# nickmass/mass-raytrace

Hardware: AMD Instinct MI355X
Metric: Msamples/sec (rays traced/sec) at 1920×1080×1024spp; 1/2/4/8-GPU scaling (higher is better)
Workload: dtype f32

## Files before the change

mass-raytrace_amd/csrc/device/layout.h:

```cpp
#pragma once
#include <stdint.h>

#include "nf_bound.h"

namespace mrt {

enum : uint32_t { KIND_BOX = 1, KIND_SPHERE = 2, KIND_TRI = 3, KIND_INST = 4, KIND_MODEL = 5, KIND_VOLUME = 6 };
constexpr uint32_t kBoxFlag = 0x80000000u;
enum : uint32_t { kVolInstance = 1, kVolModel = 2 };
constexpr uint32_t kLdsTag = 0x40000000u;
constexpr uint32_t kIdxMask = 0x3FFFFFFFu;
constexpr uint32_t KIND_END = 0;
enum : uint32_t { TRI_FLAG_ALPHA = 1u, TRI_FLAG_UV = 2u, TRI_FLAG_EVE = 4u };
constexpr uint32_t kTriAlpha = 0x80000000u;
constexpr uint32_t kTriIdMask = 0x0FFFFFFFu;

constexpr uint32_t kNfIdx = 0x0FFFFFFFu;
constexpr uint32_t kNfForceL = 0x10000000u, kNfForceR = 0x20000000u;
constexpr uint32_t kNfPop = 0x0FFFFFFFu;
constexpr int kNfExpMin = -100;
constexpr uint32_t kNfStack = 25u;
constexpr uint32_t kNfWildFew = 16u;
constexpr uint32_t kNoParent = 0xFFFFFFFFu;
constexpr uint32_t kWorldKey = 0x80000000u;
enum : uint32_t { VNF_SPHERE = 0, VNF_TRI = 1, VNF_INST = 2, VNF_MODEL = 3 };

constexpr uint32_t SURF_PROGRAM = 0xFFu;
constexpr uint32_t kSurfStack = 4;
struct GpuSurfOp {
  uint32_t op, tex, arg, pad;
  float color[4];
};
struct GpuSurfRef {
  uint32_t kind, index, len, pad;
  float color[4];
};

struct GpuMaterial {
  uint32_t kind, surf_kind, texture;
  float param;
  float color[4];
  uint32_t left, right;
  uint32_t surf_len;
  uint32_t pad1;
};

constexpr uint32_t kTexBlockW = 8, kTexBlockH = 4;
struct GpuTexture {
  uint32_t width, height, wrap;
  uint32_t offset;
};
MRT_HD uint32_t texel_index(uint32_t tpr, uint32_t x, uint32_t y) {
  return (((y >> 2) * tpr + (x >> 3)) << 5) + ((y & 3u) << 3) + (x & 7u);
}

constexpr uint32_t kTriShadeQuads = 7;

constexpr uint32_t kEveQuads = 5;

struct DevScene {
  const uint32_t* slots;
  uint32_t world_begin, world_end;
  const float* inst_inv;
  const float* inst_fwd;
  const uint32_t* inst_mat;
  const uint32_t* model_mat;
  const float* sph;
  const uint32_t* sph_mat;
  const float* tri_shade;
  const GpuMaterial* materials;
  const GpuTexture* textures;
  const uint32_t* texels;
  uint32_t fast_ok;
  uint32_t n_slots, n_tris, n_sph, n_inst, n_models, n_materials, n_textures, n_texels;
  uint32_t* dbg;
  const float* vol_nid;
  const uint32_t* vol_mat;
  const float* ln_table;
  uint32_t n_vol;
  const GpuSurfOp* surf_ops;
  uint32_t n_surf_ops;
  uint32_t bg_kind;
  float bg_color[4];
  const GpuSurfRef* bg_faces;
  const float* bg_m;
  const uint32_t* slots_tl;
  const uint32_t* tlet;
  uint32_t n_tlet;
  uint32_t tl_world_begin;
  uint32_t nf_ok, nf_world;
  uint32_t nf_wild_root;
  const uint32_t* vnf_leaf;
  uint32_t vnf_base[4];
  uint32_t n_vnf;
  NfBound nfb;
  const float* eve;
  const float* tri_tb;
  uint32_t n_eve;
};

}
```

mass-raytrace_amd/csrc/device/material.h:

```cpp
#pragma once
#include "walk.h"

namespace mrt {

struct Surf {
  V3 point, normal;
  V2 uv;
  bool has_uv, front_face;
  uint32_t material;
};

#if defined(__HIP_DEVICE_COMPILE__)
#define MRT_PIN_LOAD(x) asm volatile("" : "+v"(x))
#else
#define MRT_PIN_LOAD(x) (void)0
#endif

struct EveTex {
  uint32_t normal_occlusion, albedo_roughness, pmdg;
};
MRT_HD const float* eve_record(const DevScene& S, uint32_t rec) {
  return S.eve + (size_t)MRT_IDX(S, rec, S.n_eve, 25) * (kEveQuads * 4);
}
MRT_HD EveTex load_eve_tex(const DevScene& S, uint32_t rec) {
  const float4 q = *reinterpret_cast<const float4*>(eve_record(S, rec));
  return EveTex{f2u(q.x), f2u(q.y), f2u(q.z)};
}
MRT_HD V3 eve_tangent_normal(const DevScene& S, uint32_t rec, V2 uv, LocalCounters& lc) {
  const V4 px = texture_get_f(S, load_eve_tex(S, rec).normal_occlusion, uv, lc);
  const float py = px.y * 2.0f - 1.0f, pw = px.w * 2.0f - 1.0f;
  const float x = (1.0f - py * py) - pw * pw;
  return unit(V3{py, pw, sqrtf(fabsf(x))});
}

template <bool EXT>
MRT_HD Surf resolve_hit(const DevScene& S, V3 o, V3 d, const Hit& h, LocalCounters& lc) {
  Surf s;
  V3 ro = o, rd = d;
  const uint32_t ckind = h.container >> 28, cidx = h.container & 0x0FFFFFFFu;
  V3 f0, f1, f2, f3;
  uint32_t over = MRT_NO_MATERIAL;
  if (ckind == MRT_REF_INSTANCE) {
    V3 c0, c1, c2, c3;
    over = S.inst_mat[MRT_IDX(S, cidx, S.n_inst, 12)];
    load_m12(S.inst_inv + (size_t)MRT_IDX(S, cidx, S.n_inst, 9) * 12, c0, c1, c2, c3);
    ro = xform(c0, c1, c2, c3, o, 1.0f);
    rd = xform(c0, c1, c2, c3, d, 0.0f);
  } else if (ckind == MRT_REF_MODEL) {
    over = S.model_mat[MRT_IDX(S, cidx, S.n_models, 13)];
  }
  const uint32_t pkind = h.prim >> 28, pidx = h.prim & 0x0FFFFFFFu;
  V3 outward;
  s.point = ro + rd * h.t;
  if (pkind == MRT_REF_VOLUME) {
    s.normal = V3{1.0f, 0.0f, 0.0f};
    s.front_face = true;
    s.has_uv = false;
    s.uv = V2{0, 0};
    s.material = S.vol_mat[MRT_IDX(S, pidx, S.n_vol, 16)];
    return s;
  }
  if (pkind == MRT_REF_SPHERE) {
    const uint32_t sp = MRT_IDX(S, pidx, S.n_sph, 10);
    V3 c = ld3(S.sph + (size_t)sp * 4);
    float r = S.sph[(size_t)sp * 4 + 3];
    s.material = S.sph_mat[sp];
    MRT_PIN_LOAD(s.material);
    outward = (s.point - c) / r;
    s.has_uv = false;
    s.uv = V2{0, 0};
  } else {
    TriShade t = load_tri(S, pidx);
    float4 tq{}, bq{};
    if (EXT && S.tri_tb) {
      const float4* tb = reinterpret_cast<const float4*>(S.tri_tb) + (size_t)MRT_IDX(S, pidx, S.n_tris, 3) * 2;
      tq = tb[0], bq = tb[1];
    }
    float a0, a1, a2;
    tri_bary(t, s.point, a0, a1, a2);
    outward = (t.na * a0 + t.nb * a1) + t.nc * a2;
    s.has_uv = (t.flags & TRI_FLAG_UV) != 0;
    s.uv = uv_or_zero(s.has_uv, (t.uva * a0 + t.uvb * a1) + t.uvc * a2);
    s.material = t.material;
    if (EXT && S.tri_tb && s.has_uv && (t.flags & TRI_FLAG_EVE)) {
      const V3 tn = eve_tangent_normal(S, t.eve, s.uv, lc);
      outward = ((V3{tq.x, tq.y, tq.z} * tn.x) + (V3{bq.x, bq.y, bq.z} * tn.y)) + (outward * tn.z);
    }
  }
  s.front_face = dot(rd, outward) < 0.0f;
  s.normal = s.front_face ? outward : -outward;
  if (ckind == MRT_REF_INSTANCE) {
    load_m12(S.inst_fwd + (size_t)MRT_IDX(S, cidx, S.n_inst, 11) * 12, f0, f1, f2, f3);
    s.point = xform(f0, f1, f2, f3, s.point, 1.0f);
    s.normal = unit(xform(f0, f1, f2, f3, s.normal, 0.0f));
  }
  if (over != MRT_NO_MATERIAL) s.material = over;
  return s;
}
MRT_HD Surf resolve_hit(const DevScene& S, V3 o, V3 d, const Hit& h) {
  LocalCounters lc;
  return resolve_hit<false>(S, o, d, h, lc);
}

MRT_DEV V3 random_in_unit_sphere(PathRng& rng) {
  for (;;) {
    float x = rng.f32() * 2.0f - 1.0f;
    float y = rng.f32() * 2.0f - 1.0f;
    float z = rng.f32() * 2.0f - 1.0f;
    V3 v{x, y, z};
    if (length_squared(v) >= 1.0f) continue;
    return v;
  }
}
MRT_DEV V3 random_in_unit_disk(PathRng& rng) {
  for (;;) {
    float x = rng.f32() * 2.0f - 1.0f;
    float y = rng.f32() * 2.0f - 1.0f;
    V3 v{x, y, 0.0f};
    if (length_squared(v) >= 1.0f) continue;
    return v;
  }
}

MRT_DEV float reflectance(float cosine, float ref_idx) {
  float r0 = (1.0f - ref_idx) / (1.0f + ref_idx);
  r0 = r0 * r0;
  float x = 1.0f - cosine;
  return r0 + (1.0f - r0) * (x * ((x * x) * (x * x)));
}

struct DevCamera {
  V3 origin, llc, horizontal, vertical, u, v;
  float lens_radius;
};

MRT_DEV void camera_ray_uv(const DevCamera& cam, float u, float v, PathRng& rng, V3& o, V3& d) {
  V3 blur = random_in_unit_disk(rng) * cam.lens_radius;
  V3 offset = cam.u * blur.x + cam.v * blur.y;
  o = cam.origin + offset;
  d = (((cam.llc + (cam.horizontal * u)) + (cam.vertical * v)) - cam.origin) - offset;
}

MRT_DEV void camera_ray(const DevCamera& cam, uint32_t x, uint32_t y, uint32_t W, uint32_t H, PathRng& rng, V3& o,
                        V3& d) {
  float u = ((float)x + rng.f32()) / (float)(W - 1);
  float v = ((float)y + rng.f32()) / (float)(H - 1);
  camera_ray_uv(cam, u, v, rng, o, d);
}

template <bool EXT>
MRT_DEV V3 background(const DevScene& S, V3 d, LocalCounters& lc) {
  if (S.bg_kind == MRT_BG_SOLID) return V3{S.bg_color[0], S.bg_color[1], S.bg_color[2]};
  if (S.bg_kind == MRT_BG_SKY) {
    V3 ud = unit(d);
    float t = 0.5f * (ud.y + 1.0f);
    return (fill3(1.0f) * (1.0f - t)) + (V3{0.5f, 0.7f, 1.0f} * t);
  }
  V2 uv{0.0f, 0.0f};
  uint32_t face = 0;
  if (!EXT || S.bg_kind == MRT_BG_SKYSPHERE) {
    V3 p = unit(d);
    float theta = acosf(p.y);
    float phi = atan2f(p.z * -1.0f, p.x) + kPi;
    uv = V2{phi / (2.0f * kPi), theta / kPi};
  } else if (EXT) {
    const float* mf = S.bg_m;
    const M4 m{V4{mf[0], mf[1], mf[2], mf[3]}, V4{mf[4], mf[5], mf[6], mf[7]}, V4{mf[8], mf[9], mf[10], mf[11]},
               V4{mf[12], mf[13], mf[14], mf[15]}};
    V3 p = transform(m, d, 0.0f);
    V3 a{fabsf(p.x), fabsf(p.y), fabsf(p.z)};
    float max_axis = 0.0f, u = 0.0f, v = 0.0f;
    if (a.x >= a.y && a.x >= a.z) {
      if (p.x > 0.0f) face = 0, u = p.z * -1.0f, v = p.y;
      else face = 1, u = p.z, v = p.y;
      max_axis = a.x;
    } else if (a.y >= a.x && a.y >= a.z) {
      if (p.y > 0.0f) face = 3, u = p.x, v = p.z * -1.0f;
      else face = 2, u = p.x, v = p.z;
      max_axis = a.y;
    } else if (a.z >= a.x && a.z >= a.y) {
      if (p.z > 0.0f) face = 4, u = p.x, v = p.y;
      else face = 5, u = p.x * -1.0f, v = p.y;
      max_axis = a.z;
    }
    uv = V2{0.5f * (u / max_axis + 1.0f), 0.5f * (v / max_axis + 1.0f)};
  }
  const GpuSurfRef f = S.bg_faces[face];
  V4 px = surface_ref_get_f<EXT>(S, f.kind, f.index, f.len, f.color, uv, lc);
  return V3{px.x, px.y, px.z};
}

struct MatHead {
  uint32_t kind, surf_kind, texture;
  float param;
  float color[4];
};
MRT_DEV MatHead load_mat_head(const DevScene& S, uint32_t mi) {
  const GpuMaterial* p = S.materials + MRT_IDX(S, mi, S.n_materials, 4);
  return MatHead{p->kind, p->surf_kind, p->texture, p->param, {p->color[0], p->color[1], p->color[2], p->color[3]}};
}
MRT_DEV uint32_t mix_pick(const DevScene& S, uint32_t mi, MatHead& m, PathRng& rng) {
  while (m.kind == MRT_MAT_MIX) {
    const GpuMaterial* p = S.materials + MRT_IDX(S, mi, S.n_materials, 4);
    const uint32_t left = p->left, right = p->right;
    mi = rng.f32() < m.param ? left : right;
    m = load_mat_head(S, mi);
  }
  return mi;
}
template <bool EXT>
MRT_DEV V4 mat_get_f(const DevScene& S, const MatHead& m, uint32_t mi, V2 uv, LocalCounters& lc) {
  uint32_t len = 0;
  if (EXT && m.surf_kind == SURF_PROGRAM) len = S.materials[MRT_IDX(S, mi, S.n_materials, 4)].surf_len;
  return surface_ref_get_f<EXT>(S, m.surf_kind, m.texture, len, m.color, uv, lc);
}

template <bool EXT>
MRT_DEV void lambertian(const DevScene& S, const MatHead& m, uint32_t mi, const Surf& s, PathRng& rng, V3& atten,
                        V3& new_d, LocalCounters& lc) {
  V3 dir = s.normal + unit(random_in_unit_sphere(rng));
  if (near_zero(dir)) dir = s.normal;
  V4 c = mat_get_f<EXT>(S, m, mi, uv_or_zero(s.has_uv, s.uv), lc);
  atten = V3{c.x, c.y, c.z};
  new_d = dir;
}

template <bool EXT>
MRT_DEV bool scatter(const DevScene& S, const Surf& s, V3 d, PathRng& rng, V3& emitted, V3& atten, V3& new_d,
                     LocalCounters& lc, uint32_t& root_kind) {
  const MatHead root = load_mat_head(S, s.material);
  root_kind = root.kind;
  emitted = V3{0, 0, 0};
  uint32_t pmdg_rec = 0xFFFFFFFFu;
  V4 pmdg{};
  {
    MatHead e = root;
    mix_pick(S, s.material, e, rng);
    if (e.kind == MRT_MAT_DIFFUSE_LIGHT) emitted = V3{e.color[0], e.color[1], e.color[2]};
    if (EXT && e.kind == MRT_MAT_EVE && s.has_uv) {
      pmdg_rec = e.texture;
      pmdg = texture_get_f(S, load_eve_tex(S, pmdg_rec).pmdg, s.uv, lc);
      const float* g = eve_record(S, pmdg_rec) + 16;
      emitted = (V3{g[0], g[1], g[2]} * pmdg.w) * 10.0f;
    }
  }
  MatHead m = root;
  const uint32_t mi = mix_pick(S, s.material, m, rng);
  V2 uv = uv_or_zero(s.has_uv, s.uv);
  if (EXT && m.kind == MRT_MAT_EVE) {
    if (!s.has_uv) return false;
    const uint32_t rec = m.texture;
    const EveTex tex = load_eve_tex(S, rec);
    const V4 ar = texture_get_f(S, tex.albedo_roughness, s.uv, lc);
    if (rec != pmdg_rec) pmdg = texture_get_f(S, tex.pmdg, s.uv, lc);
    const V3 albedo{ar.x, ar.y, ar.z};
    const float roughness = ar.w, paint = pmdg.x, dirt = pmdg.z;
    const float i = pmdg.y * 3.0f;
    uint32_t i0 = f2usize(floorf(i)), i1 = f2usize(ceilf(i));
    i0 = i0 < 3u ? i0 : 3u;
    i1 = i1 < 3u ? i1 : 3u;
    const float t = i - (float)i0;
    const float* pal = eve_record(S, rec) + 4;
    const V3 mc = (ld3(pal + 3 * i0) * (1.0f - t)) + (ld3(pal + 3 * i1) * t);
    const V3 color = ((((albedo * mc) * (1.0f - paint)) + (albedo * paint)) * (1.0f - fminf(dirt, 1.0f))) +
                     (V3{0.01f, 0.005f, 0.0f} * dirt);
    const float ratio = fminf(roughness + dirt, 1.0f);
    m = MatHead{rng.f32() < ratio ? MRT_MAT_LAMBERTIAN : MRT_MAT_SPECULAR, MRT_SURF_SOLID, 0u, 1.8f,
                {color.x, color.y, color.z, 1.0f}};
  }
  switch (m.kind) {
    case MRT_MAT_LAMBERTIAN:
      lambertian<EXT>(S, m, mi, s, rng, atten, new_d, lc);
      return true;
    case MRT_MAT_METAL: {
      V3 reflected = reflect(unit(d), s.normal);
      V3 dir = reflected + (random_in_unit_sphere(rng) * m.param);
      if (dot(dir, s.normal) > 0.0f) {
        V4 c = mat_get_f<EXT>(S, m, mi, uv, lc);
        atten = V3{c.x, c.y, c.z};
        new_d = dir;
        return true;
      }
      return false;
// ... 30 lines not shown
```

mass-raytrace_amd/csrc/device/passes.hip:

```cpp
#include <algorithm>

#include "../host/display.h"
#include "ctx.h"
#include "display_math.h"

using namespace mrt;

namespace {

__global__ __launch_bounds__(kBlock) void k_selftest_division(unsigned long long n, unsigned long long seed,
                                                              unsigned long long* mismatches) {
  unsigned long long bad = 0;
  const unsigned long long stride = (unsigned long long)gridDim.x * kBlock;
  for (unsigned long long i = blockIdx.x * kBlock + threadIdx.x; i < n; i += stride) {
    uint64_t x = seed ^ (i * 0x9E3779B97F4A7C15ull);
    unsigned long long r1 = splitmix64_next(x), r2 = splitmix64_next(x);
    uint32_t ua = (uint32_t)r1, ub = (uint32_t)(r1 >> 32);
    switch (r2 & 7) {
      case 0:
        ub |= 0x007FFFFFu;
        break;
      case 1:
        ub &= 0xFF800000u;
        break;
// ... 49 lines not shown
#pragma unroll
  for (uint32_t step = 128; step > 0; step >>= 1)
    if (t[lo + step] <= u) lo += step;
  return lo;
}

__global__ __launch_bounds__(kBlock) void k_max_u32(const uint32_t* v, uint32_t n, uint32_t* out) {
  uint32_t m = 0;
  for (uint32_t i = blockIdx.x * kBlock + threadIdx.x; i < n; i += gridDim.x * kBlock) m = v[i] > m ? v[i] : m;
  for (int off = 32; off > 0; off >>= 1) {
    const uint32_t o = __shfl_xor(m, off, 64);
    m = o > m ? o : m;
  }
  if (lane_id() == 0) atomicMax(out, m);
}

__global__ __launch_bounds__(kBlock) void k_shard_pack(const uint32_t* pixlist, uint32_t n, const float* rgb,
                                                       const uint32_t* b, uint4* slab) {
  const uint32_t k = blockIdx.x * kBlock + threadIdx.x;
  if (k >= n) return;
  const uint32_t p = pixlist[k];
  slab[k] = make_uint4(__float_as_uint(rgb[3 * (size_t)p]), __float_as_uint(rgb[3 * (size_t)p + 1]),
                       __float_as_uint(rgb[3 * (size_t)p + 2]), b[p]);
}
__global__ __launch_bounds__(kBlock) void k_shard_unpack(const uint32_t* pixlist, uint32_t n, const uint4* slab,
                                                         float* rgb, uint32_t* b) {
  const uint32_t k = blockIdx.x * kBlock + threadIdx.x;
  if (k >= n) return;
  const uint32_t p = pixlist[k];
  const uint4 v = slab[k];
  rgb[3 * (size_t)p] = __uint_as_float(v.x);
  rgb[3 * (size_t)p + 1] = __uint_as_float(v.y);
  rgb[3 * (size_t)p + 2] = __uint_as_float(v.z);
  b[p] = v.w;
}

template <bool RNG, bool EXT>
__global__ __launch_bounds__(kBlock) void k_prepass(DevScene S, DevCamera cam, uint32_t W, uint32_t H,
                                                    unsigned long long seed, float4* ray_ro, float4* ray_rd,
                                                    float* albedo, float* normal) {
  const uint32_t p = blockIdx.x * kBlock + threadIdx.x;
  if (p >= W * H) return;
  const uint32_t y = p / W, x = p - y * W;
  PathRng rng = path_rng(seed, p, 0xFFFFFFFFu);
  V3 o, d;
  camera_ray_uv(cam, (float)x / (float)(W - 1), (float)y / (float)(H - 1), rng, o, d);
  ray_ro[p] = make_float4(o.x, o.y, o.z, 0.0f);
  ray_rd[p] = make_float4(d.x, d.y, d.z, 0.0f);
  const TravIn tin{S, reinterpret_cast<const uint4*>(S.slots), S.world_begin, ray_ro, ray_rd, kTmin};
  LocalCounters lc;
  const Hit h = closest_hit<false, RNG, EXT>(tin, p, INFINITY, lc, rng);
  V3 a{0.0f, 0.0f, 0.0f}, n{0.0f, 0.0f, 0.0f};
  if (h.prim != kRefNone) {
    Surf s = resolve_hit<EXT>(S, o, d, h, lc);
    V3 emitted, atten, nd;
    uint32_t mkind;
    a = scatter<EXT>(S, s, d, rng, emitted, atten, nd, lc, mkind) ? atten : emitted;
    n = s.normal;
  } else {
    a = background<EXT>(S, d, lc);
  }
  albedo[3 * (size_t)p] = a.x, albedo[3 * (size_t)p + 1] = a.y, albedo[3 * (size_t)p + 2] = a.z;
  normal[3 * (size_t)p] = n.x, normal[3 * (size_t)p + 1] = n.y, normal[3 * (size_t)p + 2] = n.z;
}

template <bool RNG, bool EXT>
__global__ __launch_bounds__(kBlock) void k_shade_rays(DevScene S, const float* rays, uint32_t n, float tmin,
                                                       float tmax, unsigned long long seed, float4* ray_ro,
                                                       float4* ray_rd, mrt_shade_out* out) {
  const uint32_t i = blockIdx.x * kBlock + threadIdx.x;
  if (i >= n) return;
  const float* r = rays + 6 * (size_t)i;
  const V3 o{r[0], r[1], r[2]}, d{r[3], r[4], r[5]};
  ray_ro[i] = make_float4(o.x, o.y, o.z, 0.0f);
  ray_rd[i] = make_float4(d.x, d.y, d.z, 0.0f);
  PathRng rng = path_rng(seed, i, 0xFFFFFFFDu);
  const TravIn tin{S, reinterpret_cast<const uint4*>(S.slots), S.world_begin, ray_ro, ray_rd, tmin};
  LocalCounters lc;
  const Hit h = closest_hit<false, RNG, EXT>(tin, i, tmax, lc, rng);
  mrt_shade_out w{};
  if (h.prim != kRefNone) {
    const Surf s = resolve_hit<EXT>(S, o, d, h, lc);
    V3 emitted, atten{0, 0, 0}, nd{0, 0, 0};
    uint32_t mkind;
    const bool cont = scatter<EXT>(S, s, d, rng, emitted, atten, nd, lc, mkind);
    w.prim = h.prim, w.container = h.container, w.t = h.t;
    w.flags = (s.front_face ? MRT_SHADE_FRONT_FACE : 0u) | (s.has_uv ? MRT_SHADE_HAS_UV : 0u) |
              (cont ? MRT_SHADE_SCATTERED : 0u);
    w.point[0] = s.point.x, w.point[1] = s.point.y, w.point[2] = s.point.z;
    w.normal[0] = s.normal.x, w.normal[1] = s.normal.y, w.normal[2] = s.normal.z;
    w.uv[0] = s.has_uv ? s.uv.x : 0.0f, w.uv[1] = s.has_uv ? s.uv.y : 0.0f;
    w.material = s.material;
    w.emitted[0] = emitted.x, w.emitted[1] = emitted.y, w.emitted[2] = emitted.z;
    if (cont) {
      w.attenuation[0] = atten.x, w.attenuation[1] = atten.y, w.attenuation[2] = atten.z;
      w.direction[0] = nd.x, w.direction[1] = nd.y, w.direction[2] = nd.z;
    }
  }
  out[i] = w;
}

__global__ __launch_bounds__(kBlock) void k_tonemap(uint32_t W, uint32_t H, const float* rgb, const uint32_t* b,
                                                    uint32_t passes, uint32_t mode, const uint32_t* max_count,
                                                    const uint32_t* g, uint8_t* out) {
  const uint32_t p = blockIdx.x * kBlock + threadIdx.x;
  if (p >= W * H) return;
  const uint32_t y = p / W, x = p - y * W;
  uint8_t* dst = out + ((size_t)(H - 1 - y) * W + x) * 3;
  if (mode == MRT_DISPLAY_ALBEDO || mode == MRT_DISPLAY_NORMAL) {
#pragma unroll
    for (int c = 0; c < 3; ++c) {
      const float v = rgb[3 * (size_t)p + c];
      if (mode == MRT_DISPLAY_NORMAL) {
        dst[c] = (uint8_t)rs_u8(((v + 1.0f) / 2.0f) * 255.0f);
      } else {
        const float q = rs_max(rs_min(v, 1.0f), 0.0f);
        dst[c] = (uint8_t)(q >= 1.0f ? 255u : gamma_byte(g, q));
      }
    }
    return;
  }
  if (passes == 0) {
    dst[0] = dst[1] = dst[2] = 0;
    return;
  }
  const float scale = 1.0f / (float)passes;
  if (mode == MRT_DISPLAY_DEPTH) {
    const uint32_t m = *max_count;
    const float max_depth = (float)(m > 1u ? m : 1u) * scale;
    const float d = rs_min(rs_max(((float)b[p] * scale) / max_depth, 0.0f), 1.0f);
    dst[0] = dst[1] = dst[2] = (uint8_t)rs_u8(d * 255.0f);
  } else {
    dst[0] = (uint8_t)gamma_byte(g, scale * rgb[3 * (size_t)p]);
    dst[1] = (uint8_t)gamma_byte(g, scale * rgb[3 * (size_t)p + 1]);
    dst[2] = (uint8_t)gamma_byte(g, scale * rgb[3 * (size_t)p + 2]);
  }
}

// ... 254 lines not shown
```

mass-raytrace_amd/csrc/device/shade.h:

```cpp
#pragma once
#include "pool.h"

namespace {

using namespace mrt;

constexpr uint32_t kShadeMiss = 0xFFFFFFFEu, kShadeIdle = 0xFFFFFFFFu;
template <bool EXT>
MRT_DEV bool shade_step(const DevScene& S, uint32_t max_depth, const Hit& h, V3& o, V3& d, V3& T, V3& L, uint32_t& k,
                        PathRng& rng, LocalCounters& lc, uint32_t& nbounce, uint32_t& mat, uint32_t& mkind) {
  if (h.prim == kRefNone) {
    mat = kShadeMiss;
    L = L + T * background<EXT>(S, d, lc);
    return false;
  }
  Surf s = resolve_hit<EXT>(S, o, d, h, lc);
  mat = s.material;
  V3 emitted, atten, nd;
  bool cont = scatter<EXT>(S, s, d, rng, emitted, atten, nd, lc, mkind);
  L = L + T * emitted;
  if (!cont) return false;
  T = T * atten;
  k += 1;
  nbounce += 1;
  o = s.point;
  d = nd;
  return k < max_depth;
}

MRT_DEV void shade_coherence(uint32_t mat, uint32_t mkind, LocalCounters& lc) {
  const unsigned long long act = __ballot(mat != kShadeIdle);
  if (act == 0) return;
  const uint32_t kind = mat == kShadeIdle ? 0xFFu : mat == kShadeMiss ? 16u : mkind;
  uint32_t nk = 0, nm = 0;
  for (uint32_t kk = 0; kk <= 16; ++kk) nk += __ballot(kind == kk) != 0;
  for (unsigned long long rem = act; rem;) {
    const uint32_t m0 = __shfl(mat, __ffsll((long long)rem) - 1, 64);
    rem &= ~__ballot(mat == m0);
    ++nm;
  }
  if (lane_id() == 0) {
    lc.shade_waves += 1;
    lc.shade_kinds += nk;
    lc.shade_materials += nm;
  }
}

}
```

mass-raytrace_amd/csrc/device/trace.hip:

```cpp
#include <string.h>

#include <algorithm>

#include "ctx.h"

using namespace mrt;

namespace {

constexpr size_t kTraceLdsMaxBytes = 160 * 1024;
constexpr uint32_t kStashQuads = 4;

template <bool COUNT, bool LDS, uint32_t ALPHA, bool RNG, int BLK, bool NF = false, bool WILD = false, bool VBLAS = false>
__global__ __launch_bounds__(BLK) __attribute__((amdgpu_waves_per_eu(NF ? (COUNT ? 1 : 5) : (ALPHA == 0 && !RNG && !COUNT ? 8 : 1)))) void k_trace(DevScene S, PathBufs in, uint4* hits, Ctrl* ctrl, uint32_t cur,
                                                  DevCounters* cnt, float tmin, float tmax, TraceTune tune) {
  static_assert(!NF || (!LDS && !RNG), "the near-first walk has no treelet and no traversal draws");
  static_assert(!WILD || NF, "only the near-first walk has a wild tree");
  static_assert(!VBLAS || RNG, "a volume draws");
  const uint32_t n = ctrl->active[cur];
  if (blockIdx.x == 0 && threadIdx.x == 0) {
    ctrl->active[cur ^ 1] = 0;
    ctrl->surv[cur ^ 1] = 0;
  }
  if (n == 0) return;
// ... 98 lines not shown
      if (RNG) trav_store_rng(tin, t);
      const Hit h = trav_hit<LDS>(tin, t);
      hits[t.ray] = make_uint4(__float_as_uint(h.t), h.prim, h.container, 0u);
      seg += 1;
      nh += t.prim != kRefNone;
      t.ray = kIdle;
    }
  }
  if (COUNT) flush_counters(cnt, lc, seg, nh, 0, 0);
}

template <bool RNG>
__global__ __launch_bounds__(kBlock) void k_trace_simple(DevScene S, PathBufs in, uint4* hits, Ctrl* ctrl,
                                                         uint32_t cur, DevCounters* cnt) {
  const uint32_t n = ctrl->active[cur];
  if (blockIdx.x == 0 && threadIdx.x == 0) {
    ctrl->active[cur ^ 1] = 0;
    ctrl->surv[cur ^ 1] = 0;
  }
  LocalCounters lc;
  uint32_t seg = 0, nh = 0;
  const TravIn tin{S, reinterpret_cast<const uint4*>(S.slots), S.world_begin, in.ro, in.rd, kTmin, in.rng};
  for (uint32_t i = blockIdx.x * kBlock + threadIdx.x; i < n; i += gridDim.x * kBlock) {
    PathRng rng{0, 0};
    if (RNG) rng = rng_unpack(in.rng[i]);
    Hit h = closest_hit<true, RNG>(tin, i, INFINITY, lc, rng);
    if (RNG) in.rng[i] = rng_pack(rng);
    hits[i] = make_uint4(__float_as_uint(h.t), h.prim, h.container, 0u);
    seg += 1;
    nh += h.prim != kRefNone;
  }
  flush_counters(cnt, lc, seg, nh, 0, 0);
}

__global__ __launch_bounds__(kBlock) void k_rays_in(const float* rays, uint32_t n, PathBufs out) {
  uint32_t i = blockIdx.x * kBlock + threadIdx.x;
  if (i >= n) return;
  const float* r = rays + 6 * (size_t)i;
  out.ro[i] = make_float4(r[0], r[1], r[2], __uint_as_float(i));
  out.rd[i] = make_float4(r[3], r[4], r[5], __uint_as_float(0u));
  out.rng[i] = rng_pack(path_rng(0, i, 0xFFFFFFFEu));
}

template <bool EXT>
__global__ __launch_bounds__(kBlock) void k_rays_out(DevScene S, PathBufs in, const uint4* hits, uint32_t n,
                                                     uint4* out) {
  uint32_t i = blockIdx.x * kBlock + threadIdx.x;
  if (i >= n) return;
  const float4 o4 = in.ro[i], d4 = in.rd[i];
  const uint4 hv = hits[i];
  Hit h{__uint_as_float(hv.x), hv.y, hv.z};
  uint32_t front = 0;
  LocalCounters lc;
  if (h.prim != kRefNone)
    front = resolve_hit<EXT>(S, V3{o4.x, o4.y, o4.z}, V3{d4.x, d4.y, d4.z}, h, lc).front_face ? 1u : 0u;
  out[i] = make_uint4(h.prim, h.container, __float_as_uint(h.prim != kRefNone ? h.t : 0.0f), front);
}

using TraceFn = void (*)(DevScene, PathBufs, uint4*, Ctrl*, uint32_t, DevCounters*, float, float, TraceTune);
TraceFn trace_kernel(bool count, bool lds, uint32_t alpha, bool rng, bool vblas, int block, bool nf, bool wild) {
  return with_value<true, false>(count, [&](auto COUNT) {
    return with_value<2u, 1u, 0u>(alpha, [&](auto ALPHA) -> TraceFn {
      if (nf)
        return with_value<true, false>(wild, [&](auto WILD) -> TraceFn { return k_trace<COUNT, false, ALPHA, false, kBlock, true, WILD>; });
      return with_value<true, false>(rng, [&](auto RNG) {
        return with_value<true, false>(vblas, [&](auto VB) {
          return with_value<true, false>(lds, [&](auto LDS) {
            return with_value<1024, 512, kBlock>(block, [&](auto B) -> TraceFn {
              return k_trace<COUNT, LDS, ALPHA, RNG, LDS ? B : kBlock, false, false, RNG && VB>;
            });
          });
        });
      });
    });
  });
}

}

uint32_t persistent_grid(mrt_ctx* c, const void* f, size_t smem, bool shared, int block, int share_num,
                         int share_den) {
  auto key = std::make_pair(f, smem);
  auto it = c->grids.find(key);
  if (it != c->grids.end()) return it->second;
  if (smem > 0) HIP_CHECK(hipFuncSetAttribute(f, hipFuncAttributeMaxDynamicSharedMemorySize, (int)kTraceLdsMaxBytes));
  int per_cu = 0;
  HIP_CHECK(hipOccupancyMaxActiveBlocksPerMultiprocessor(&per_cu, f, block, smem));
  if (shared) per_cu = std::max(1, per_cu * share_num / share_den);
  if (c->tun.wgs_per_cu) per_cu = (int)c->tun.wgs_per_cu;
  const uint32_t g = (uint32_t)c->cus * (uint32_t)std::max(1, per_cu);
  c->grids[key] = g;
  return g;
}

void launch_trace(mrt_ctx* c, hipStream_t st, const Queue& q, const PathBufs& in, uint32_t cur, bool count,
                  float tmin, float tmax) {
  const Tuning& t = c->tun;
  const bool shared = t.queues > 1;
  const uint32_t alpha = c->scene_alpha ? (c->scene_ext ? 2u : 1u) : 0u;
  const bool rng = c->facts.trav_rng, vblas = rng && c->scene_vblas;
  const bool nf = t.use_nf, wild = nf && c->S.nf_wild_root != 0;
  const bool lds = !nf && c->facts.treelet;
  const int block = lds ? t.trace_block : kBlock;
  const TraceFn f = trace_kernel(count, lds, alpha, rng, vblas, block, nf, wild);
  size_t smem;
  uint32_t grid;
  if (nf) {
    smem = (size_t)(kNfStack - (wild ? 0u : 1u)) * block * 4;
// ... 50 lines not shown
```

mass-raytrace_amd/csrc/device/upload.cpp:

```cpp
#include "upload.h"

#include <math.h>
#include <stdlib.h>
#include <string.h>

#include <algorithm>
#include <queue>
#include <stdexcept>
#include <unordered_map>

#include "records.h"

namespace mrt {

namespace {

struct SurfResolver {
  const mrt_scene_desc& d;
  HostScene& s;
  std::string& err;
  std::unordered_map<uint32_t, GpuSurfRef> memo;
  std::vector<int8_t> tex_zero_alpha;
  static constexpr uint32_t kMaxOps = 256;

// ... 359 lines not shown
      if (m.surface >= d.n_surfaces) return (err = "material surface out of range", false);
      GpuSurfRef r;
      if (!surf.resolve(m.surface, r)) return false;
      g.surf_kind = r.kind;
      g.texture = r.index;
      g.surf_len = r.len;
      for (int k = 0; k < 4; ++k) g.color[k] = r.color[k];
    } else if (m.kind == MRT_MAT_DIFFUSE_LIGHT || m.kind == MRT_MAT_ISOTROPHIC) {
      for (int k = 0; k < 3; ++k) g.color[k] = m.emit[k];
    } else if (m.kind == MRT_MAT_MIX) {
      if (m.left >= i || m.right >= i) return (err = "Mix children must precede the Mix in the material table", false);
      g.left = m.left;
      g.right = m.right;
    } else if (m.kind == MRT_MAT_EVE) {
      if (!ext || !ext->eve_materials || m.surface >= ext->n_eve_materials)
        return (err = "eve material index out of range", false);
      g.texture = m.surface;
    }
    s.materials.push_back(g);
  }
  const uint32_t n_eve = ext && ext->eve_materials ? ext->n_eve_materials : 0;
  for (uint32_t i = 0; i < n_eve; ++i) {
    const mrt_eve_material& e = ext->eve_materials[i];
    if (e.normal_occlusion >= d.n_textures || e.albedo_roughness >= d.n_textures || e.pmdg >= d.n_textures)
      return (err = "eve material texture out of range", false);
    float q[kEveQuads * 4] = {};
    const uint32_t tex[3] = {e.normal_occlusion, e.albedo_roughness, e.pmdg};
    memcpy(q, tex, 12);
    memcpy(q + 4, e.colors, 48);
    memcpy(q + 16, e.glow, 12);
    s.eve.insert(s.eve.end(), q, q + kEveQuads * 4);
  }
  for (uint32_t i = 0; i < d.n_textures; ++i) {
    const mrt_texture& t = d.textures[i];
    if (t.wrap == MRT_WRAP_MIRROR) return (err = "WrapMode::Mirror is unimplemented (texture.rs:280-282)", false);
    if (t.wrap != MRT_WRAP_REPEAT && t.wrap != MRT_WRAP_CLAMP) return (err = "bad wrap mode", false);
    if (t.width == 0 || t.height == 0 || !t.rgba) return (err = "empty texture", false);
    const uint32_t tpr = (t.width + kTexBlockW - 1) / kTexBlockW, rows = (t.height + kTexBlockH - 1) / kTexBlockH;
    const size_t n = (size_t)tpr * rows * kTexBlockW * kTexBlockH, base = s.texels.size();
    if (base + n > 0xFFFFFFFFull) return (err = "textures past 2^32 texels", false);
    GpuTexture g{t.width, t.height, t.wrap, (uint32_t)base};
    s.textures.push_back(g);
    s.texels.resize(base + n, 0u);
    for (uint32_t y = 0; y < t.height; ++y)
      for (uint32_t x = 0; x < t.width; ++x) {
        uint32_t v;
        memcpy(&v, t.rgba + 4 * ((size_t)y * t.width + x), 4);
        s.texels[base + texel_index(tpr, x, y)] = v;
      }
  }
  auto check_mat = [&](uint32_t m, bool allow_none) {
    return (allow_none && m == MRT_NO_MATERIAL) || m < d.n_materials;
  };
  for (uint32_t i = 0; i < d.n_spheres; ++i) {
    const mrt_sphere& sp = d.spheres[i];
    if (!check_mat(sp.material, false)) return (err = "sphere material out of range", false);
    for (int k = 0; k < 3; ++k) s.sph.push_back(sp.center[k]);
    s.sph.push_back(sp.radius);
    s.sph_mat.push_back(sp.material);
  }
  s.tri_shade.reserve((size_t)d.n_triangles * kTriShadeQuads * 4);
  for (uint32_t i = 0; i < d.n_triangles; ++i) {
    const mrt_triangle& t = d.triangles[i];
    if (!check_mat(t.material, false)) return (err = "triangle material out of range", false);
    float q[28] = {t.a[0],   t.a[1],   t.a[2],   t.b[0],   t.b[1],   t.b[2],   t.c[0],
                   t.c[1],   t.c[2],   t.na[0],  t.na[1],  t.na[2],  t.nb[0],  t.nb[1],
                   t.nb[2],  t.nc[0],  t.nc[1],  t.nc[2],  t.uva[0], t.uva[1], t.uvb[0],
                   t.uvb[1], t.uvc[0], t.uvc[1], 0,        0,        0,        0};
    uint32_t flags = (t.flags & MRT_TRI_HAS_UV) ? TRI_FLAG_UV : 0;
    if (d.materials[t.material].kind == MRT_MAT_EVE) {
      flags |= TRI_FLAG_EVE;
      memcpy(&q[26], &d.materials[t.material].surface, 4);
    }
    memcpy(&q[24], &t.material, 4);
    memcpy(&q[25], &flags, 4);
    s.tri_shade.insert(s.tri_shade.end(), q, q + 28);
  }
  if (!s.eve.empty()) {
    s.tri_tb.reserve((size_t)d.n_triangles * 8);
    for (uint32_t i = 0; i < d.n_triangles; ++i) {
      const mrt_triangle& t = d.triangles[i];
      const float q[8] = {t.tangent[0], t.tangent[1], t.tangent[2], 0, t.bitangent[0], t.bitangent[1], t.bitangent[2], 0};
      s.tri_tb.insert(s.tri_tb.end(), q, q + 8);
    }
  }
  for (uint32_t i = 0; i < d.n_volumes; ++i) {
    const mrt_volume& v = d.volumes[i];
    if (!check_mat(v.material, false)) return (err = "volume material out of range", false);
    s.vol_nid.push_back(-1.0f / v.density);
    s.vol_mat.push_back(v.material);
  }
  if (d.n_volumes) {
    s.ln_table.resize((size_t)1 << 23);
    for (uint32_t m = 0; m < (1u << 23); ++m) s.ln_table[m] = logf((float)m * 0x1p-23f);
  }
  for (uint32_t i = 0; i < d.n_instances; ++i) {
    const mrt_instance& in = d.instances[i];
    if (!check_mat(in.material, true)) return (err = "instance material out of range", false);
    put_m4_12(s.inst_inv, in.inv);
    put_m4_12(s.inst_fwd, in.fwd);
    s.inst_mat.push_back(in.material);
  }
  for (uint32_t i = 0; i < d.n_models; ++i) {
    if (!check_mat(d.models[i].material, true)) return (err = "model material out of range", false);
    s.model_mat.push_back(d.models[i].material);
  }
  s.bg_kind = d.background.kind;
  for (int k = 0; k < 3; ++k) s.bg_color[k] = d.background.color[k];
  if (d.background.kind == MRT_BG_SKYSPHERE || d.background.kind == MRT_BG_CUBEMAP) {
    const bool cube = d.background.kind == MRT_BG_CUBEMAP;
    for (int k = 0; k < (cube ? 6 : 1); ++k) {
      GpuSurfRef r;
      if (!surf.resolve(cube ? d.background.faces[k] : d.background.surface, r)) return false;
      s.bg_faces.push_back(r);
    }
    if (cube) memcpy(s.bg_m, d.background.transform, sizeof(s.bg_m));
  } else if (d.background.kind > MRT_BG_CUBEMAP) {
    return (err = "bad background kind", false);
  }
  s.world_begin = 0;
  for (uint32_t r = 0; r < d.n_roots; ++r)
    if (!e.emit_tree(d.roots[r], false)) return false;
  s.world_end = e.n_slots();
  e.push_end();
  std::unordered_map<uint32_t, size_t> blas;
  auto region_of = [&](uint32_t root) -> BlasRegion* {
    auto it = blas.find(root);
    if (it == blas.end()) {
      uint32_t b = e.n_slots();
      if (!e.emit_tree(MRT_REF(MRT_REF_NODE, root), true)) return nullptr;
      s.blas_regions.push_back({b, e.n_slots(), 0, false});
      it = blas.emplace(root, s.blas_regions.size() - 1).first;
      e.push_end();
    }
    return &s.blas_regions[it->second];
  };
  for (auto& p : e.jump_patches) {
    BlasRegion* r = region_of(p.second);
    if (!r) return false;
    r->refs++;
    if (rec::kind(s.slots.data(), p.first) == KIND_MODEL) r->model = true;
    rec::set_blas_range(s.slots.data(), p.first, r->begin, r->end);
  }
  for (auto& p : e.volume_patches) {
    BlasRegion* r = region_of(p.second);
    if (!r) return false;
    const uint32_t* w = s.slots.data();
    for (auto rs = std::lower_bound(s.rec_starts.begin(), s.rec_starts.end(), r->begin);
         rs != s.rec_starts.end() && *rs < r->end; ++rs)
      if (!rec::is_box(w, *rs) && rec::kind(w, *rs) != KIND_TRI)
        return (err = "a volume target's BLAS must hold triangles only", false);
    r->refs++;
    if (rec::volume_target(w, p.first) == kVolModel) r->model = true;
    rec::set_volume_blas(s.slots.data(), p.first, r->begin);
  }
  if (e.mix_alpha) s.trav_rng = true;
  if (sibling_layout) relayout(s);
  if (!build_nf_trees(d, s, err)) return false;
// ... 104 lines not shown
```

mass-raytrace_amd/csrc/device/upload.h:

```cpp
#pragma once
#include <string>
#include <vector>

#include "../../../include/massrt.h"
#include "layout.h"

namespace mrt {

struct BlasRegion {
  uint32_t begin, end, refs;
  bool model;
};

struct HostScene {
  std::vector<uint32_t> slots;
  std::vector<uint32_t> rec_starts;
  uint32_t world_begin = 0, world_end = 0;
  std::vector<float> inst_inv, inst_fwd;
  std::vector<uint32_t> inst_mat, model_mat;
  std::vector<float> sph;
  std::vector<uint32_t> sph_mat;
  std::vector<float> tri_shade;
  std::vector<float> eve;
  std::vector<float> tri_tb;
  std::vector<GpuMaterial> materials;
  std::vector<GpuTexture> textures;
  std::vector<uint32_t> texels;
  uint32_t fast_ok = 1;
  uint32_t early_ok = 1;
  bool has_alpha = false;
  bool trav_rng = false;
  bool vol_blas = false;
  std::vector<float> vol_nid;
  std::vector<uint32_t> vol_mat;
  std::vector<float> ln_table;
  std::vector<GpuSurfOp> surf_ops;
  uint32_t bg_kind = 0;
  float bg_color[4] = {0, 0, 0, 0};
  std::vector<GpuSurfRef> bg_faces;
  float bg_m[16] = {0};
  std::vector<BlasRegion> blas_regions;
  std::vector<uint32_t> tlet, slots_tl;
  uint32_t tl_world_begin = 0, tl_boxes = 0;
  uint32_t n_box_records = 0, n_prim_records = 0, max_depth = 0;
  bool nf_ok = false;
  uint32_t nf_world = 0, nf_boxes = 0, nf_stack_need = 0, nf_first_slot = 0;
  std::vector<uint32_t> vnf_leaf;
  uint32_t vnf_base[4] = {0, 0, 0, 0};
  std::string nf_note;
  NfBound nfb{};
  uint32_t nf_wild = 0;
  uint32_t nf_wild_root = 0;
  uint32_t nf_cones = 0;
  bool keep_nf_boxes = false;
  int nf_build = 2;
  std::vector<float> nf_leaf_box;
  std::vector<uint8_t> nf_inst_wild;
};

enum { kNfBuildNever = 0, kNfBuildAlways = 1, kNfBuildAuto = 2 };

enum : unsigned {
  kArrNullIfEmpty = 1,
  kArrDeviceOnly = 2,
};
template <typename F>
void for_each_scene_array(const HostScene& s, F&& f) {
  auto vec = [&](auto field, const auto& v, unsigned flags = 0) { f(field, v.data(), v.size() * sizeof(v[0]), flags); };
  vec(&DevScene::slots, s.slots);
  vec(&DevScene::slots_tl, s.slots_tl, kArrDeviceOnly);
  vec(&DevScene::tlet, s.tlet, kArrDeviceOnly);
  vec(&DevScene::inst_inv, s.inst_inv);
  vec(&DevScene::inst_fwd, s.inst_fwd);
  vec(&DevScene::inst_mat, s.inst_mat);
  vec(&DevScene::model_mat, s.model_mat);
  vec(&DevScene::sph, s.sph);
  vec(&DevScene::sph_mat, s.sph_mat);
  vec(&DevScene::tri_shade, s.tri_shade);
  vec(&DevScene::materials, s.materials);
  vec(&DevScene::textures, s.textures);
  vec(&DevScene::texels, s.texels);
  vec(&DevScene::vol_nid, s.vol_nid);
  vec(&DevScene::vol_mat, s.vol_mat);
  vec(&DevScene::ln_table, s.ln_table, kArrNullIfEmpty);
  vec(&DevScene::surf_ops, s.surf_ops);
  vec(&DevScene::bg_faces, s.bg_faces);
  f(&DevScene::bg_m, &s.bg_m[0], sizeof(s.bg_m), 0u);
  vec(&DevScene::vnf_leaf, s.vnf_leaf);
  vec(&DevScene::eve, s.eve);
  vec(&DevScene::tri_tb, s.tri_tb, kArrNullIfEmpty);
}

struct ScenePlan {
  std::vector<size_t> off;
  size_t total = 0;
};
inline ScenePlan plan_scene(const HostScene& s) {
  ScenePlan p;
  for_each_scene_array(s, [&](auto, const void*, size_t bytes, unsigned) {
    p.off.push_back(p.total);
    p.total += (bytes + 255) & ~(size_t)255;
  });
  return p;
}

inline DevScene host_dev_scene(const HostScene& s) {
  DevScene S{};
  for_each_scene_array(s, [&](auto field, auto* data, size_t bytes, unsigned flags) {
    if (!(flags & kArrDeviceOnly)) S.*field = bytes || !(flags & kArrNullIfEmpty) ? data : nullptr;
  });
  S.world_begin = s.world_begin;
  S.world_end = s.world_end;
  S.fast_ok = (s.fast_ok ? 1u : 0u) | (s.early_ok ? 2u : 0u);
  S.n_slots = (uint32_t)(s.slots.size() / 4);
  S.n_tris = (uint32_t)(s.tri_shade.size() / (kTriShadeQuads * 4));
  S.n_sph = (uint32_t)s.sph_mat.size();
  S.n_inst = (uint32_t)s.inst_mat.size();
  S.n_models = (uint32_t)s.model_mat.size();
  S.n_materials = (uint32_t)s.materials.size();
  S.n_textures = (uint32_t)s.textures.size();
  S.n_texels = (uint32_t)s.texels.size();
  S.n_vol = (uint32_t)s.vol_nid.size();
  S.n_surf_ops = (uint32_t)s.surf_ops.size();
  S.bg_kind = s.bg_kind;
  for (int k = 0; k < 4; ++k) S.bg_color[k] = s.bg_color[k];
  S.nf_ok = s.nf_ok ? 1u : 0u;
  S.nf_world = s.nf_world;
  S.nf_wild_root = s.nf_ok ? s.nf_wild_root : 0u;
  for (int k = 0; k < 4; ++k) S.vnf_base[k] = s.vnf_base[k];
  S.n_vnf = (uint32_t)(s.vnf_leaf.size() / 2);
  S.nfb = s.nfb;
  S.n_eve = (uint32_t)(s.eve.size() / (kEveQuads * 4));
  return S;
}

bool build_nf_trees(const mrt_scene_desc& d, HostScene& s, std::string& err);

bool build_host_scene(const mrt_scene_desc& d, HostScene& out, std::string& err, bool sibling_layout = true,
                      const mrt_scene_ext* ext = nullptr, const mrt_volume_target* targets = nullptr,
                      uint32_t n_targets = 0);

void build_treelet(HostScene& s, uint32_t budget);

}
```

Measured before the change: 1323.

## Embed material headers in sphere records and per-instance/model head arrays

Sphere records become 64-byte structs holding center, radius, material id and a copy of the material header (kinds, texture, param, color), so the non-extended resolve path gets the root material without a dependent load from the materials array. Instances and models also get precomputed header arrays for their override materials. Scatter uses the prefetched header when present. This removes a dependent gather per hit at the cost of a larger sphere footprint (16 to 64 bytes) and duplicated material data.

```diff
diff --git a/mass-raytrace_amd/csrc/device/layout.h b/mass-raytrace_amd/csrc/device/layout.h
--- a/mass-raytrace_amd/csrc/device/layout.h
+++ b/mass-raytrace_amd/csrc/device/layout.h
@@ -56,6 +56,11 @@
 
 constexpr uint32_t kTriShadeQuads = 7;
 
+constexpr uint32_t kSphQuads = 3, kSphStride = 4;
+MRT_HD uint32_t sph_pack_kinds(uint32_t kind, uint32_t surf_kind) { return kind | (surf_kind << 8); }
+
+constexpr uint32_t kHeadQuads = 2;
+
 constexpr uint32_t kEveQuads = 5;
 
 struct DevScene {
@@ -65,8 +70,9 @@
   const float* inst_fwd;
   const uint32_t* inst_mat;
   const uint32_t* model_mat;
-  const float* sph;
-  const uint32_t* sph_mat;
+  const float* inst_head;
+  const float* model_head;
+  const float* sph_rec;
   const float* tri_shade;
   const GpuMaterial* materials;
   const GpuTexture* textures;
diff --git a/mass-raytrace_amd/csrc/device/material.h b/mass-raytrace_amd/csrc/device/material.h
--- a/mass-raytrace_amd/csrc/device/material.h
+++ b/mass-raytrace_amd/csrc/device/material.h
@@ -33,13 +33,29 @@
   return unit(V3{py, pw, sqrtf(fabsf(x))});
 }
 
-template <bool EXT>
-MRT_HD Surf resolve_hit(const DevScene& S, V3 o, V3 d, const Hit& h, LocalCounters& lc) {
+struct MatHead {
+  uint32_t kind, surf_kind, texture;
+  float param;
+  float color[4];
+};
+struct RootHead {
+  MatHead m;
+  bool has;
+};
+MRT_HD MatHead over_head(const float* heads, uint32_t i) {
+  const float4* p = reinterpret_cast<const float4*>(heads) + (size_t)i * kHeadQuads;
+  const float4 q0 = p[0], q1 = p[1];
+  return MatHead{f2u(q0.x), f2u(q0.y), f2u(q0.z), q0.w, {q1.x, q1.y, q1.z, q1.w}};
+}
+
+template <bool EXT>
+MRT_HD Surf resolve_hit(const DevScene& S, V3 o, V3 d, const Hit& h, LocalCounters& lc, RootHead& root) {
   Surf s;
   V3 ro = o, rd = d;
   const uint32_t ckind = h.container >> 28, cidx = h.container & 0x0FFFFFFFu;
   V3 f0, f1, f2, f3;
   uint32_t over = MRT_NO_MATERIAL;
+  root.has = false;
   if (ckind == MRT_REF_INSTANCE) {
     V3 c0, c1, c2, c3;
     over = S.inst_mat[MRT_IDX(S, cidx, S.n_inst, 12)];
@@ -61,11 +77,20 @@
     return s;
   }
   if (pkind == MRT_REF_SPHERE) {
-    const uint32_t sp = MRT_IDX(S, pidx, S.n_sph, 10);
-    V3 c = ld3(S.sph + (size_t)sp * 4);
-    float r = S.sph[(size_t)sp * 4 + 3];
-    s.material = S.sph_mat[sp];
-    MRT_PIN_LOAD(s.material);
+    const float4* rec = reinterpret_cast<const float4*>(S.sph_rec) + (size_t)MRT_IDX(S, pidx, S.n_sph, 10) * kSphStride;
+    const float4 cr = rec[0];
+    float4 q0 = rec[1];
+    MRT_PIN_LOAD(q0.w);
+    s.material = f2u(q0.w);
+    if (!EXT) {
+      float4 q1 = rec[2];
+      MRT_PIN_LOAD(q1.x);
+      const uint32_t kinds = f2u(q0.x);
+      root.m = MatHead{kinds & 0xFFu, kinds >> 8, f2u(q0.y), q0.z, {q1.x, q1.y, q1.z, q1.w}};
+      root.has = true;
+    }
+    const V3 c{cr.x, cr.y, cr.z};
+    const float r = cr.w;
     outward = (s.point - c) / r;
     s.has_uv = false;
     s.uv = V2{0, 0};
@@ -89,17 +114,23 @@
   }
   s.front_face = dot(rd, outward) < 0.0f;
   s.normal = s.front_face ? outward : -outward;
+  if (over != MRT_NO_MATERIAL) s.material = over;
+  if (!EXT && over != MRT_NO_MATERIAL) {
+    root.m = ckind == MRT_REF_INSTANCE ? over_head(S.inst_head, MRT_IDX(S, cidx, S.n_inst, 26))
+                                       : over_head(S.model_head, MRT_IDX(S, cidx, S.n_models, 27));
+    root.has = true;
+  }
   if (ckind == MRT_REF_INSTANCE) {
     load_m12(S.inst_fwd + (size_t)MRT_IDX(S, cidx, S.n_inst, 11) * 12, f0, f1, f2, f3);
     s.point = xform(f0, f1, f2, f3, s.point, 1.0f);
     s.normal = unit(xform(f0, f1, f2, f3, s.normal, 0.0f));
   }
-  if (over != MRT_NO_MATERIAL) s.material = over;
   return s;
 }
 MRT_HD Surf resolve_hit(const DevScene& S, V3 o, V3 d, const Hit& h) {
   LocalCounters lc;
-  return resolve_hit<false>(S, o, d, h, lc);
+  RootHead root;
+  return resolve_hit<false>(S, o, d, h, lc, root);
 }
 
 MRT_DEV V3 random_in_unit_sphere(PathRng& rng) {
@@ -190,11 +221,6 @@
   return V3{px.x, px.y, px.z};
 }
 
-struct MatHead {
-  uint32_t kind, surf_kind, texture;
-  float param;
-  float color[4];
-};
 MRT_DEV MatHead load_mat_head(const DevScene& S, uint32_t mi) {
   const GpuMaterial* p = S.materials + MRT_IDX(S, mi, S.n_materials, 4);
   return MatHead{p->kind, p->surf_kind, p->texture, p->param, {p->color[0], p->color[1], p->color[2], p->color[3]}};
@@ -226,9 +252,9 @@
 }
 
 template <bool EXT>
-MRT_DEV bool scatter(const DevScene& S, const Surf& s, V3 d, PathRng& rng, V3& emitted, V3& atten, V3& new_d,
-                     LocalCounters& lc, uint32_t& root_kind) {
-  const MatHead root = load_mat_head(S, s.material);
+MRT_DEV bool scatter(const DevScene& S, const Surf& s, const RootHead& rh, V3 d, PathRng& rng, V3& emitted, V3& atten,
+                     V3& new_d, LocalCounters& lc, uint32_t& root_kind) {
+  const MatHead root = rh.has ? rh.m : load_mat_head(S, s.material);
   root_kind = root.kind;
   emitted = V3{0, 0, 0};
   uint32_t pmdg_rec = 0xFFFFFFFFu;
diff --git a/mass-raytrace_amd/csrc/device/passes.hip b/mass-raytrace_amd/csrc/device/passes.hip
--- a/mass-raytrace_amd/csrc/device/passes.hip
+++ b/mass-raytrace_amd/csrc/device/passes.hip
@@ -125,10 +125,11 @@
   const Hit h = closest_hit<false, RNG, EXT>(tin, p, INFINITY, lc, rng);
   V3 a{0.0f, 0.0f, 0.0f}, n{0.0f, 0.0f, 0.0f};
   if (h.prim != kRefNone) {
-    Surf s = resolve_hit<EXT>(S, o, d, h, lc);
+    RootHead root;
+    Surf s = resolve_hit<EXT>(S, o, d, h, lc, root);
     V3 emitted, atten, nd;
     uint32_t mkind;
-    a = scatter<EXT>(S, s, d, rng, emitted, atten, nd, lc, mkind) ? atten : emitted;
+    a = scatter<EXT>(S, s, root, d, rng, emitted, atten, nd, lc, mkind) ? atten : emitted;
     n = s.normal;
   } else {
     a = background<EXT>(S, d, lc);
@@ -153,10 +154,11 @@
   const Hit h = closest_hit<false, RNG, EXT>(tin, i, tmax, lc, rng);
   mrt_shade_out w{};
   if (h.prim != kRefNone) {
-    const Surf s = resolve_hit<EXT>(S, o, d, h, lc);
+    RootHead root;
+    const Surf s = resolve_hit<EXT>(S, o, d, h, lc, root);
     V3 emitted, atten{0, 0, 0}, nd{0, 0, 0};
     uint32_t mkind;
-    const bool cont = scatter<EXT>(S, s, d, rng, emitted, atten, nd, lc, mkind);
+    const bool cont = scatter<EXT>(S, s, root, d, rng, emitted, atten, nd, lc, mkind);
     w.prim = h.prim, w.container = h.container, w.t = h.t;
     w.flags = (s.front_face ? MRT_SHADE_FRONT_FACE : 0u) | (s.has_uv ? MRT_SHADE_HAS_UV : 0u) |
               (cont ? MRT_SHADE_SCATTERED : 0u);
diff --git a/mass-raytrace_amd/csrc/device/shade.h b/mass-raytrace_amd/csrc/device/shade.h
--- a/mass-raytrace_amd/csrc/device/shade.h
+++ b/mass-raytrace_amd/csrc/device/shade.h
@@ -14,10 +14,11 @@
     L = L + T * background<EXT>(S, d, lc);
     return false;
   }
-  Surf s = resolve_hit<EXT>(S, o, d, h, lc);
+  RootHead root;
+  Surf s = resolve_hit<EXT>(S, o, d, h, lc, root);
   mat = s.material;
   V3 emitted, atten, nd;
-  bool cont = scatter<EXT>(S, s, d, rng, emitted, atten, nd, lc, mkind);
+  bool cont = scatter<EXT>(S, s, root, d, rng, emitted, atten, nd, lc, mkind);
   L = L + T * emitted;
   if (!cont) return false;
   T = T * atten;
diff --git a/mass-raytrace_amd/csrc/device/trace.hip b/mass-raytrace_amd/csrc/device/trace.hip
--- a/mass-raytrace_amd/csrc/device/trace.hip
+++ b/mass-raytrace_amd/csrc/device/trace.hip
@@ -174,8 +174,9 @@
   Hit h{__uint_as_float(hv.x), hv.y, hv.z};
   uint32_t front = 0;
   LocalCounters lc;
+  RootHead root;
   if (h.prim != kRefNone)
-    front = resolve_hit<EXT>(S, V3{o4.x, o4.y, o4.z}, V3{d4.x, d4.y, d4.z}, h, lc).front_face ? 1u : 0u;
+    front = resolve_hit<EXT>(S, V3{o4.x, o4.y, o4.z}, V3{d4.x, d4.y, d4.z}, h, lc, root).front_face ? 1u : 0u;
   out[i] = make_uint4(h.prim, h.container, __float_as_uint(h.prim != kRefNone ? h.t : 0.0f), front);
 }
 
diff --git a/mass-raytrace_amd/csrc/device/upload.cpp b/mass-raytrace_amd/csrc/device/upload.cpp
--- a/mass-raytrace_amd/csrc/device/upload.cpp
+++ b/mass-raytrace_amd/csrc/device/upload.cpp
@@ -435,12 +435,24 @@
   auto check_mat = [&](uint32_t m, bool allow_none) {
     return (allow_none && m == MRT_NO_MATERIAL) || m < d.n_materials;
   };
+  auto push_head = [&](std::vector<float>& out, uint32_t m) {
+    float q[kHeadQuads * 4] = {};
+    if (m != MRT_NO_MATERIAL) memcpy(q, &s.materials[m], sizeof(q));
+    out.insert(out.end(), q, q + kHeadQuads * 4);
+  };
+  s.sph_rec.reserve((size_t)d.n_spheres * kSphStride * 4);
   for (uint32_t i = 0; i < d.n_spheres; ++i) {
     const mrt_sphere& sp = d.spheres[i];
     if (!check_mat(sp.material, false)) return (err = "sphere material out of range", false);
-    for (int k = 0; k < 3; ++k) s.sph.push_back(sp.center[k]);
-    s.sph.push_back(sp.radius);
-    s.sph_mat.push_back(sp.material);
+    const GpuMaterial& g = s.materials[sp.material];
+    if (g.kind > 0xFFu || g.surf_kind > 0xFFu) return (err = "material kind does not fit a sphere record", false);
+    float q[kSphStride * 4] = {sp.center[0], sp.center[1], sp.center[2], sp.radius};
+    const uint32_t q0[2] = {sph_pack_kinds(g.kind, g.surf_kind), g.texture};
+    memcpy(q + 4, q0, 8);
+    memcpy(q + 6, &g.param, 4);
+    memcpy(q + 7, &sp.material, 4);
+    memcpy(q + 8, g.color, 16);
+    s.sph_rec.insert(s.sph_rec.end(), q, q + kSphStride * 4);
   }
   s.tri_shade.reserve((size_t)d.n_triangles * kTriShadeQuads * 4);
   for (uint32_t i = 0; i < d.n_triangles; ++i) {
@@ -483,10 +495,12 @@
     put_m4_12(s.inst_inv, in.inv);
     put_m4_12(s.inst_fwd, in.fwd);
     s.inst_mat.push_back(in.material);
+    push_head(s.inst_head, in.material);
   }
   for (uint32_t i = 0; i < d.n_models; ++i) {
     if (!check_mat(d.models[i].material, true)) return (err = "model material out of range", false);
     s.model_mat.push_back(d.models[i].material);
+    push_head(s.model_head, d.models[i].material);
   }
   s.bg_kind = d.background.kind;
   for (int k = 0; k < 3; ++k) s.bg_color[k] = d.background.color[k];
diff --git a/mass-raytrace_amd/csrc/device/upload.h b/mass-raytrace_amd/csrc/device/upload.h
--- a/mass-raytrace_amd/csrc/device/upload.h
+++ b/mass-raytrace_amd/csrc/device/upload.h
@@ -18,8 +18,8 @@
   uint32_t world_begin = 0, world_end = 0;
   std::vector<float> inst_inv, inst_fwd;
   std::vector<uint32_t> inst_mat, model_mat;
-  std::vector<float> sph;
-  std::vector<uint32_t> sph_mat;
+  std::vector<float> inst_head, model_head;
+  std::vector<float> sph_rec;
   std::vector<float> tri_shade;
   std::vector<float> eve;
   std::vector<float> tri_tb;
@@ -74,8 +74,9 @@
   vec(&DevScene::inst_fwd, s.inst_fwd);
   vec(&DevScene::inst_mat, s.inst_mat);
   vec(&DevScene::model_mat, s.model_mat);
-  vec(&DevScene::sph, s.sph);
-  vec(&DevScene::sph_mat, s.sph_mat);
+  vec(&DevScene::inst_head, s.inst_head);
+  vec(&DevScene::model_head, s.model_head);
+  vec(&DevScene::sph_rec, s.sph_rec);
   vec(&DevScene::tri_shade, s.tri_shade);
   vec(&DevScene::materials, s.materials);
   vec(&DevScene::textures, s.textures);
@@ -114,7 +115,7 @@
   S.fast_ok = (s.fast_ok ? 1u : 0u) | (s.early_ok ? 2u : 0u);
   S.n_slots = (uint32_t)(s.slots.size() / 4);
   S.n_tris = (uint32_t)(s.tri_shade.size() / (kTriShadeQuads * 4));
-  S.n_sph = (uint32_t)s.sph_mat.size();
+  S.n_sph = (uint32_t)(s.sph_rec.size() / (kSphStride * 4));
   S.n_inst = (uint32_t)s.inst_mat.size();
   S.n_models = (uint32_t)s.model_mat.size();
   S.n_materials = (uint32_t)s.materials.size();
```

New measurement: 1326, median of 6. No clear change (+0.2%).
